# Kaz-K/medical-image-editing

Hardware: AMD Instinct MI355X
Metric: images/sec (train step, 256x256 2D slices) (higher is better)
Workload: dtype f32

## Files before the change

### medical-image-editing_amd/csrc/conv_common.h

```cpp
#pragma once
#include "common.h"
#include <cstdlib>

inline int conv_max_blocks() {
    static const int v = [] {
        const char* e = getenv("VQW_CONV_MAX_BLOCKS");
        const int b = e ? atoi(e) : 256;
        return b < 8 ? 8 : (b > 256 ? 256 : b);
    }();
    return v;
}

inline int conv_slab_split(int nsp, int nblk, int max_slabs, int* kt_out) {
    int nsb = conv_max_blocks() / nblk;
    if (nsb > max_slabs) nsb = max_slabs;
    if (nsb > nsp) nsb = nsp;
    if (nsb < 1) nsb = 1;
    const int kt = (nsp + nsb - 1) / nsb;
    if (kt_out) *kt_out = kt;
    return (nsp + kt - 1) / kt;
}
inline int conv_region_runs(int nsp, int ntn, int wg_per_cu) {
    int groups = conv_max_blocks() * wg_per_cu / ntn;
    if (groups < 1) groups = 1;
    const int even = (nsp + groups - 1) / groups;
    return even < 1 ? 1 : even;
}

struct ConvIn {
    const float* src0;
    const float* src1;
    int C0, C1, up0;
};

#ifdef __HIPCC__
static __device__ inline void collapse_up_element(const float* __restrict__ w, float* __restrict__ wc, float* __restrict__ wd, long i, int Cout, int Cin) {
    const long nfwd = 4L * Cout * 4 * Cin;
    if (i < nfwd) {
            int ci = (int)(i % Cin);
            long r = i / Cin;
            int ab = (int)(r % 4);
            r /= 4;
            int co = (int)(r % Cout);
            int par = (int)(r / Cout);
            int py = par >> 1, px = par & 1, a = ab >> 1, b = ab & 1;
            int ky0 = (py == 0) ? (a == 0 ? 0 : 1) : (a == 0 ? 0 : 2), ky1 = (py == 0) ? (a == 0 ? 0 : 2) : (a == 0 ? 1 : 2);
            int kx0 = (px == 0) ? (b == 0 ? 0 : 1) : (b == 0 ? 0 : 2), kx1 = (px == 0) ? (b == 0 ? 0 : 2) : (b == 0 ? 1 : 2);
            float acc = 0.f;
            for (int ky = ky0; ky <= ky1; ++ky)
                for (int kx = kx0; kx <= kx1; ++kx) acc += w[(((long)co * 3 + ky) * 3 + kx) * Cin + ci];
            wc[i] = acc;
        } else {
            long k = i - nfwd;
            int co = (int)(k % Cout);
            long r = k / Cout;
            int rs = (int)(r % 16);
            int ci = (int)(r / 16);
            int rr = rs >> 2, ss = rs & 3;
            int ky0 = rr == 0 ? 2 : (rr == 1 ? 1 : 0), ky1 = rr == 0 ? 2 : (rr == 1 ? 2 : (rr == 2 ? 1 : 0));
            int kx0 = ss == 0 ? 2 : (ss == 1 ? 1 : 0), kx1 = ss == 0 ? 2 : (ss == 1 ? 2 : (ss == 2 ? 1 : 0));
            float acc = 0.f;
            for (int ky = ky0; ky <= ky1; ++ky)
                for (int kx = kx0; kx <= kx1; ++kx) acc += w[(((long)co * 3 + ky) * 3 + kx) * Cin + ci];
            wd[k] = acc;
        }
}
// ... 142 lines not shown
```

### medical-image-editing_amd/csrc/conv_dil.hip

```cpp
#include "common.h"
#include "conv_common.h"
#include "mfma_util.h"

int g_dil_mode = 0;

namespace {

struct DilArgs {
    const float* x;
    const float* w;
    const float* bias;
    float* y;
    int N, H, W, Cout, dil;
    int per, total;
    int relu;
    unsigned nbx, nbw, nby;
    float* stats;
};

template <int NW, bool ACC>
__global__ void __launch_bounds__(64 * NW, 1) k_conv_dilrow(DilArgs a) {
    constexpr int NT = 64 * NW, WMAX = 32 * NW, KP = 36;
    constexpr int SLOT = (WMAX + 1) * KP;
    constexpr int WBUF = 9 * 32 * KP;
    constexpr int LH = WMAX * 8 / NT;
    constexpr int WF = 9 * 32 * 8, LW = (WF + NT - 1) / NT;
    static_assert(LH * NT == WMAX * 8, "row float4s must divide over the threads");

    extern __shared__ __attribute__((aligned(16))) float smem[];
    float* Hs = smem;
    float* Ws = smem + 3 * SLOT;
    float* Rs = Ws + WBUF;

    const int tid = threadIdx.x, lane = tid & 63, wv = tid >> 6;
    const int H = a.H, W = a.W, Cout = a.Cout, d = a.dil;
    const __amdgpu_buffer_rsrc_t rsx = make_rsrc(a.x, a.nbx), rsw = make_rsrc(a.w, a.nbw), rsy = make_rsrc(a.y, a.nby);

    const int t0 = blockIdx.x * a.per;
    const int nsteps = min(a.per, a.total - t0);
    if (nsteps <= 0) return;

    if (tid < 3 * KP) Hs[(tid / KP) * SLOT + WMAX * KP + tid % KP] = 0.f;
#pragma unroll
    for (int j = 0; j < LW; ++j) {
        const int f = tid + j * NT;
        const bool ok = (WF % NT == 0) || f < WF;
        const int row = ok ? f / 8 : 0, c4 = f % 8;
        const int tap = row / 32, n = row % 32;
        const float4 v = buf_ld4(rsw, (ok && n < Cout) ? (((unsigned)n * 9 + tap) * 32 + c4 * 4) * 4u : a.nbw);
        if (ok) *(float4*)&Ws[row * KP + c4 * 4] = v;
    }

    const unsigned row_bytes = (unsigned)W * 128u;
    unsigned h_off[LH];
    int h_lds[LH];
#pragma unroll
    for (int j = 0; j < LH; ++j) {
        const int f = tid + j * NT;
        h_off[j] = f < W * 8 ? (unsigned)f * 16u : 0xFFFFFFFFu;
        h_lds[j] = (f >> 3) * KP + (f & 7) * 4;
    }
    float4 rh[LH];
    auto issue_h = [&](int j, int g) {
        const bool ok = (g >= 0) & (h_off[j] != 0xFFFFFFFFu);
        rh[j] = buf_ld4(rsx, sel_u32(ok, (unsigned)g * row_bytes + h_off[j], a.nbx));
    };
    auto commit_h = [&](int j, int slot_f) { *(float4*)&Hs[slot_f + h_lds[j]] = rh[j]; };
    int hn, hrho, hy;
    if (t0 == 0) {
        hn = -1; hrho = d - 1; hy = -1;
    } else {
        const int Ls = H + d;
        hn = (t0 - 1) / Ls;
        int u = (t0 - 1) - hn * Ls;
        hrho = 0;
        for (;;) {
            const int L = (H - hrho + d - 1) / d;
            if (u < L) { hy = hrho + u * d; break; }
            if (u == L) { hy = -1; break; }
            u -= L + 1;
            ++hrho;
        }
    }
    auto head_row = [&]() { return (hy >= 0 && hn >= 0 && hn < a.N) ? hn * H + hy : -1; };
    auto head_next = [&]() {
        if (hy < 0) {
            if (++hrho == d) { hrho = 0; ++hn; }
            hy = hrho;
        } else {
            hy += d;
            if (hy >= H) hy = -1;
        }
    };

    int g0 = -1, g1 = -1;
#pragma unroll
    for (int s = 0; s < 3; ++s) {
        const int g = head_row();
#pragma unroll
        for (int j = 0; j < LH; ++j) issue_h(j, g);
#pragma unroll
        for (int j = 0; j < LH; ++j) commit_h(j, s * SLOT);
        head_next();
        g0 = g1;
        g1 = g;
    }
    int sA = 0, sB = SLOT, sC = 2 * SLOT;
    __syncthreads();

    const int lrow = lane & 31, lk = (lane >> 5) * 4;
    auto col_of = [&](int kx) {
        const int x = wv * 32 + lrow + (kx - 1) * d;
        return ((unsigned)x < (unsigned)W ? x : WMAX) * KP + lk;
    };
    const int cx0 = col_of(0), cx1 = col_of(1), cx2 = col_of(2);
    const float* Wb = Ws + lrow * KP + lk;

    const int co = lane & 31;
    const float bv0 = (a.bias && co < Cout) ? a.bias[co] : 0.f;
    const bool st_ok = (co < Cout) & (wv * 32 < W);
    const int col0 = 4 * (lane >> 5);
    const float lo = a.relu ? 0.f : -__builtin_inff();
    f32x16 acc, done;
    float yold[ACC ? 16 : 1];
    bool pending = false;
    int dg = 0;
    auto flush_piece = [&](int half) {
        const unsigned base = (((unsigned)dg * W + (unsigned)(wv * 32 + col0)) * (unsigned)Cout + (unsigned)co) * 4u;
        const int voff = (int)sel_u32(pending & st_ok, base, a.nby);
#pragma unroll
        for (int r8 = 0; r8 < 8; ++r8) {
            const int r = half * 8 + r8;
            const int col = (r & 3) + 8 * (r >> 2);
            __builtin_amdgcn_raw_buffer_store_b32(__float_as_uint(done[r]), rsy, voff, col * Cout * 4, 0);
        }
    };
    const int nwr = W / 32;

    for (int i = 0; i < nsteps; ++i) {
        const int g2 = (i + 2 <= nsteps) ? head_row() : -1;
        if (g0 >= 0) {
#pragma unroll
            for (int r = 0; r < 16; ++r) acc[r] = 0.f;
            constexpr int NG = 36;
            float4 av[2], bv[2];
            auto ldfrag = [&](int g, int s) {
                const int tap = g / 4, kg = g % 4, ky = tap / 3, kx = tap % 3;
                av[s] = *(const float4*)&Hs[(ky == 0 ? sA : ky == 1 ? sB : sC) + (kx == 0 ? cx0 : kx == 1 ? cx1 : cx2) + kg * 8];
                bv[s] = *(const float4*)&Wb[tap * 32 * KP + kg * 8];
            };
            auto slot = [&](int m) {
                if (m < 2) flush_piece(m);
                else if (m < 2 + LH) issue_h(m - 2, g2);
                else if (ACC && m < 2 + LH + 16) {
                    const int r = m - 2 - LH;
                    const unsigned base = (((unsigned)g0 * W + (unsigned)(wv * 32 + col0)) * (unsigned)Cout + (unsigned)co) * 4u;
                    yold[r] = __uint_as_float(__builtin_amdgcn_raw_buffer_load_b32(rsy, (int)sel_u32(st_ok, base, a.nby),
                                                                                 ((r & 3) + 8 * (r >> 2)) * Cout * 4, 0));
                }
                else if (m >= 96 && m < 96 + LH) commit_h(m - 96, sA);
            };
            auto slotted = [&](int m0) { return m0 >= 0 && (m0 < 2 + LH + (ACC ? 16 : 0) || (m0 + 4 > 96 && m0 < 96 + LH)); };
            ldfrag(0, 0);
#pragma unroll
            for (int g = 0; g < NG; ++g) {
                const int s = g & 1;
                if (g + 1 < NG) ldfrag(g + 1, s ^ 1);
                const int m0 = (g - 1) * 4;
                const bool slt = slotted(m0);
                acc = MFMA32(av[s].x, bv[s].x, acc);
                if (slt) { slot(m0); __builtin_amdgcn_sched_barrier(0); }
                acc = MFMA32(av[s].y, bv[s].y, acc);
                if (slt) { slot(m0 + 1); __builtin_amdgcn_sched_barrier(0); }
                acc = MFMA32(av[s].z, bv[s].z, acc);
                if (slt) { slot(m0 + 2); __builtin_amdgcn_sched_barrier(0); }
                acc = MFMA32(av[s].w, bv[s].w, acc);
                if (slt) { slot(m0 + 3); __builtin_amdgcn_sched_barrier(0); }
                if (!slt) {
                    __builtin_amdgcn_sched_group_barrier(0x100, 2, 0);
                    __builtin_amdgcn_sched_group_barrier(0x008, 4, 0);
                }
                if (g == 11) __syncthreads();
            }
            pending = false;
#pragma unroll
            for (int r = 0; r < 16; ++r) done[r] = fmaxf(acc[r] + bv0, lo) + (ACC ? yold[r] : 0.f);
            pending = true;
            dg = g0;
            if (a.stats) {
                float vals[16], s1, s2;
#pragma unroll
                for (int r = 0; r < 16; ++r) vals[r] = done[r];
                lane_stats<16>(vals, s1, s2);
                stat_merge_eq(s1, s2, __shfl_xor(s1, 32, 64), __shfl_xor(s2, 32, 64), 1.f / 32.f);
                if (lane < 32) { Rs[(wv * 32 + lane) * 2] = s1; Rs[(wv * 32 + lane) * 2 + 1] = s2; }
            }
        } else {
#pragma unroll
            for (int j = 0; j < LH; ++j) issue_h(j, g2);
#pragma unroll
            for (int j = 0; j < LH; ++j) commit_h(j, sA);
        }
        __syncthreads();
        if (a.stats && g0 >= 0 && tid < 32 && tid < Cout) {
            float s1 = Rs[tid * 2], s2 = Rs[tid * 2 + 1];
            for (int r = 1; r < nwr; ++r) stat_merge(s1, s2, (float)(32 * r), Rs[(r * 32 + tid) * 2], Rs[(r * 32 + tid) * 2 + 1], 32.f);
            float* o = a.stats + ((size_t)g0 * Cout + tid) * 2;
            o[0] = s1;
            o[1] = s2;
        }
        const int t = sA; sA = sB; sB = sC; sC = t;
        g0 = g1; g1 = g2;
        head_next();
    }
    flush_piece(0);
    flush_piece(1);
}


struct DilWgArgs {
    const float* x;
    const float* dy;
    float* part;
    int N, H, W, Cout, dil;
    int per, total;
    unsigned nbx, nbd;
};

template <int NW>
__global__ void __launch_bounds__(64 * NW, 1) k_conv_dilrow_wgrad(DilWgArgs a) {
    constexpr int NT = 64 * NW, WMAX = 32 * NW;
    constexpr int LH = WMAX * 8 / NT;
    extern __shared__ __attribute__((aligned(16))) float smem[];
    float* Xs = smem;

// ... 230 lines not shown
```

### medical-image-editing_amd/csrc/conv_wino64.hip

```cpp
#include "common.h"
#include "conv_common.h"
#include "mfma_util.h"
#include "wino_common.h"

extern int g_wino_mode;

namespace {

struct W64Args {
    const float* x;
    const float* u;
    const float* bias;
    float* y;
    int N, H, W, Cin, Cout;
    int tilesY, tilesX, nsp;
    int ntn, nch;
    int kt;
    int relu;
    unsigned nbx, nbu, nby;
    float* stats;
    const float* mask;
    const float* mr;
    int in_relu;
    float* y2;
// ... 43 lines not shown
    float* Rs = Ex + G::EXF;

    const int tid = threadIdx.x, lane = tid & 63;
    const int wv = __builtin_amdgcn_readfirstlane(tid >> 6);
    const int mb = wv & (NMB - 1), h = wv / NMB;
    const int H = a.H, W = a.W, Cin = a.Cin, Cout = a.Cout;
    const __amdgpu_buffer_rsrc_t rsx = make_rsrc(a.x, a.nbx), rsu = make_rsrc(a.u, a.nbu), rsy = make_rsrc(a.y, a.nby);
    const __amdgpu_buffer_rsrc_t rsm = make_rsrc((EPI == 1 || EPI == 3) ? a.mask : a.y, a.nby);
    const __amdgpu_buffer_rsrc_t rsr = make_rsrc(EPI == 3 ? a.mr : a.y, EPI == 3 ? (unsigned)((size_t)a.N * a.Cout * 8) : a.nby);
    const __amdgpu_buffer_rsrc_t rsy2 = make_rsrc(EPI == 4 ? a.y2 : a.y, EPI == 4 ? a.nby2 : a.nby);

    const int nch = a.nch;
    const wino::RegionRun run = wino::region_run(a.ntn, a.kt, a.nsp);
    const int co_base = run.tile_n * NCO;
    const int my_tiles = run.my_tiles;
    if (my_tiles <= 0) return;

    const int c4 = tid & 1;
    const wino::PitchedPix pixel = {a.img_px, a.rowb_px, a.rpx, a.ppx, a.n_sh, a.n_m};
    Halo hs;
    hs.init(tid, pixel);
    auto region_offsets = [&](int n, int tx, int ty) { hs.region_offsets(n, ty * G::TR - 1, tx * RW - 1, H, W, Cin); };
    const int u_n = (tid >> 1) & (NCO - 1);
    const int u_swz = (u_n >> 3) & 1;
    const int u_c4 = c4 ^ u_swz;
    const unsigned u_voff = (((unsigned)(tid >> 1) / NCO * Cout + co_base + u_n) * 8u + u_c4 * 4) * 4u;
    const unsigned u_jstride = (unsigned)(NT / 2 / NCO) * Cout * 32u;
    const unsigned u_cstride = 16u * Cout * 32u;
    const int u_wave = wv * 256;

    auto issue_h = [&](int j, int chunk) { hs.issue_h(rsx, j, chunk); };
    auto commit_h = [&](int j, float* Hb) { hs.commit_h(j, Hb); };
    auto issue_u = [&](int j, int chunk, float* Ub) {
        wino::buf_ld4_lds(rsu, Ub + u_wave + j * (NT * 4), u_voff, chunk * u_cstride + j * u_jstride);
    };

    int cn, ctx, cty, ch = 0;
    region_start(run.sp0, a.tilesY, a.tilesX, cn, ctx, cty);
    auto advance = [&](int& n, int& tx, int& ty, int& c) {
        const int adv = c + 1 == nch ? 1 : 0;
        c = adv ? 0 : c + 1;
        region_step(adv, a.tilesY, a.tilesX, n, tx, ty);
    };
    int n1 = cn, tx1 = ctx, ty1 = cty, ch1 = 0;
    advance(n1, tx1, ty1, ch1);
    int n2 = n1, tx2 = tx1, ty2 = ty1, ch2 = ch1;
    advance(n2, tx2, ty2, ch2);
    auto shift = [&]() {
        cn = n1; ctx = tx1; cty = ty1; ch = ch1;
        n1 = n2; tx1 = tx2; ty1 = ty2; ch1 = ch2;
        advance(n2, tx2, ty2, ch2);
    };

    const int m = lane & 15, q = lane >> 4;
    const int rA = h ? 3 : 0, rB = h ? 2 : 1, rC = h ? 1 : 2;
    const int prow = RW == 32 ? 2 * MBW * mb : 2 * (2 * mb + (m >> 3)), pcol = RW == 32 ? 2 * m : 2 * (m & 7);
    constexpr int MBW_STEP = 2 * HWS * W6_KPH;
    const int a_A = opaque(((prow + rA) * HWS + pcol) * W6_KPH + 2 * q);
    const int a_B = opaque(((prow + rB) * HWS + pcol) * W6_KPH + 2 * q);
    const int a_C = opaque(((prow + rC) * HWS + pcol) * W6_KPH + 2 * q);
    const int b_swz = ((q >> 1) ^ (m >> 3)) * 4 + (q & 1) * 2;
    const int b_0 = opaque(((h ? 3 : 0) * 4 * NCO + m) * 8 + b_swz);
    const int b_1 = opaque(((h ? 2 : 1) * 4 * NCO + m) * 8 + b_swz);
    const float sg = opaque_f(h ? -1.f : 1.f), mone = opaque_f(-1.f);

    f32x4 acc[8][MBW][NBW];
    f32x2 bf[2][NBW];
// ... 15 lines not shown
            else e[t][1][c] = __builtin_fmaf(sg, dC, dB);
        } else {
            const int k = o - 16, lr = k >> 3, t = (k >> 2) & 1, cc = k & 3;
            const float e0 = e[t][lr][0], e1 = e[t][lr][1], e2 = e[t][lr][2], e3 = e[t][lr][3];
            v[par][w][t][lr * 4 + cc] = wino::bt_row_plain(cc, e0, e1, e2, e3);
        }
    };
    auto xform_slot = [&](const float* Hn, int par, int p) {
        constexpr int NOPS = 32 * MBW, P0 = MBW == 1 ? 32 : 4;
        auto op = [&](int g) { xform_op(par, g >> 5, g & 31); };
        auto rd = [&](int g) {
            if ((g & 31) < 16 && ((g & 31) & 3) == 0) read_col(Hn, g >> 5, (g & 31) >> 2);
        };
        if (p + 3 - P0 >= 0 && p + 3 - P0 < NOPS) rd(p + 3 - P0);
        if (p - P0 >= 0 && p - P0 < NOPS && p < 64) {
            const int g = p - P0;
            if (P0 + NOPS <= 64 || g < NOPS - 2 * (P0 + NOPS - 64)) op(g);
            else { const int d = g - (NOPS - 2 * (P0 + NOPS - 64)); op(NOPS - 2 * (P0 + NOPS - 64) + 2 * d); op(NOPS - 2 * (P0 + NOPS - 64) + 2 * d + 1); }
        }
    };

    region_offsets(cn, ctx, cty);
#pragma unroll
    for (int j = 0; j < LH; ++j) issue_h(j, 0);
#pragma unroll
    for (int j = 0; j < LU; ++j) issue_u(j, 0, Us);
#pragma unroll
    for (int j = 0; j < LH; ++j) commit_h(j, Hs);
    region_offsets(n1, tx1, ty1);
#pragma unroll
    for (int j = 0; j < LH; ++j) issue_h(j, ch1);
#pragma unroll
    for (int j = 0; j < LH; ++j) commit_h(j, Hs + HBUF);
    wino::dma_wait();
    __syncthreads();
#pragma unroll
    for (int w = 0; w < MBW; ++w)
#pragma unroll
        for (int o = 0; o < 32; ++o) {
            if (o < 16 && (o & 3) == 0) read_col(Hs, w, o >> 2);
            xform_op(0, w, o);
        }
    __syncthreads();
    region_offsets(n2, tx2, ty2);

    float bvv[NBW / 2];
#pragma unroll
    for (int i = 0; i < NBW / 2; ++i) bvv[i] = a.bias ? a.bias[co_base + (h * (NBW / 2) + i) * 16 + m] : 0.f;
    const float lo = a.relu ? 0.f : -__builtin_inff();
    const bool plain = a.bias == nullptr && !a.relu;
    int spar = 0;

    auto body = [&](auto PAR, auto FIRST) {
        constexpr int par = decltype(PAR)::value;
        constexpr bool first = decltype(FIRST)::value;
        const float* Uc = Us + par * UBUF;
        const float* Hn = Hs + (par ^ 1) * HBUF;
        float* Hw = Hs + par * HBUF;
        float* Uw = Us + (par ^ 1) * UBUF;
        auto ldb = [&](int l, int nb) {
            bf[l & 1][nb] = *(const f32x2*)&Uc[(l < 4 ? b_0 : b_1) + ((l & 3) * NCO + nb * 16) * 8];
        };
        static_assert(par == 0 || (par ^ 1) == 0, "a region's last item (odd) loads U into buffer 0: buffer 1 is the epilogue's exchange area");
        auto slot = [&](int p) {
            if (p >= 1 && p < HP0 && (p - 1) % W6_ULS == 0) issue_u((p - 1) / W6_ULS, ch1, Uw);
            if (p >= HP0 && p < HP0 + LH * W6_LS && (p - HP0) % W6_LS == 0) issue_h((p - HP0) / W6_LS, ch2);
            if (p >= W6_CP && p < W6_CP + LH) commit_h(p - W6_CP, Hw);
// ... 175 lines not shown
        if (a.stats && lane < 16) {
#pragma unroll
            for (int i = 0; i < NBW / 2; ++i) {
                float* R = Rs + spar * (NMB * NCO * 2) + (mb * NCO + (hh * (NBW / 2) + i) * 16 + lane) * 2;
                R[0] = st1[i];
                R[1] = st2[i];
            }
        }
    };
    auto fold_stats = [&]() {
        if (!a.stats) return;
        if (tid < NCO) {
            const float* R = Rs + spar * (NMB * NCO * 2) + tid * 2;
            float s1 = R[0], s2 = R[1];
            constexpr float PW = 64.f * MBW;
            if (EPI == 3) {
#pragma unroll
                for (int r = 1; r < NMB; ++r) { s1 += R[r * NCO * 2]; s2 += R[r * NCO * 2 + 1]; }
            } else {
#pragma unroll
                for (int r = 1; r < NMB; ++r) stat_merge(s1, s2, PW * r, R[r * NCO * 2], R[r * NCO * 2 + 1], PW);
            }
            const int t = (cn * a.tilesX + ctx) * a.tilesY + cty;
            float* o = a.stats + ((size_t)t * Cout + co_base + tid) * 2;
            o[0] = s1;
            o[1] = s2;
        }
        spar ^= 1;
    };

    using wino::P0;
    using wino::P1;
    auto item_end = [&]() {
        wino::dma_wait();
        __syncthreads();
    };
    for (int reg = 0; reg < my_tiles; ++reg) {
        body(P0{}, std::true_type{});
        item_end();
        shift();
        body(P1{}, std::false_type{});
        item_end();
        for (int c = 2; c < nch; c += 2) {
            shift();
            if (ch2 == 0) region_offsets(n2, tx2, ty2);
            body(P0{}, std::false_type{});
            item_end();
            shift();
            body(P1{}, std::false_type{});
            item_end();
        }
        flush();
        if (h == 0) epi_send(P0{}); else epi_send(P1{});
        __syncthreads();
        if (h == 0) epi_finish(P0{}); else epi_finish(P1{});
        __syncthreads();
        fold_stats();
        shift();
        if (ch2 == 0) region_offsets(n2, tx2, ty2);
    }
}

}

static int wino64_shape(int Cin, int Cout, int W) {
    if (Cin % 16 != 0) return 0;
    if (Cout % 64 == 0) return 1;
// ... 450 lines not shown
```

### medical-image-editing_amd/csrc/conv_wino_up.hip

```cpp
#include "common.h"
#include "conv_common.h"
#include "mfma_util.h"
#include "wino_common.h"

namespace {

__device__ __host__ constexpr int up_row(int s) { return s == 2 ? 3 : s; }

__global__ void k_wino_up_weights(const float* __restrict__ w, float* __restrict__ uf, float* __restrict__ ud, int Cout, int Cin,
                                  float* __restrict__ wc, float* __restrict__ wd) {
    if (wc) {
        const long nc = 32L * Cout * Cin;
        for (long i = (long)blockIdx.x * blockDim.x + threadIdx.x; i < nc; i += (long)gridDim.x * blockDim.x) collapse_up_element(w, wc, wd, i, Cout, Cin);
    }
    const long n = (long)Cout * Cin;
    for (long e = (long)blockIdx.x * blockDim.x + threadIdx.x; e < n; e += (long)gridDim.x * blockDim.x) {
        const int co = (int)(e / Cin), ci = (int)(e % Cin);
        double g[3][3];
        for (int ky = 0; ky < 3; ++ky)
            for (int kx = 0; kx < 3; ++kx) g[ky][kx] = (double)w[(((long)co * 3 + ky) * 3 + kx) * Cin + ci];
        for (int flip = 0; flip < 2; ++flip) {
            double gf[3][3], u[4][4];
            for (int ky = 0; ky < 3; ++ky)
                for (int kx = 0; kx < 3; ++kx) gf[ky][kx] = flip ? g[2 - ky][2 - kx] : g[ky][kx];
// ... 8 lines not shown
                        const double ci_ = (i == 0 ? 1.0 : i == 1 ? 2.0 : -1.0), cj_ = (j == 0 ? 1.0 : j == 1 ? 2.0 : -1.0);
                        ud[((((long)(co >> 3) * 9 + xi) * Cin + ci) * 8) + (co & 7)] = (float)(ci_ * cj_ * u[i][j]);
                    }
                }
        }
    }
}

constexpr int WU_KPH = 10;

struct WUpDgArgs {
    const float* dy;
    const float* u;
    float* g;
    int N, H, W, Cin, Cout;
    int tilesY, tilesX, nsp, ntn, nch, kt;
    unsigned nbd, nbu, nbg;
};

template <int NBW, bool ACC>
__global__ void __launch_bounds__(512, 1) k_conv_wino_up_dgrad(WUpDgArgs a) {
    constexpr int NT = 512, NCO = 16 * NBW;
    constexpr int RW = 32, TR = 16, HR = TR + 2, HWV = RW + 2, HWS = 34;
    constexpr int HBUF = HR * HWS * WU_KPH;
    constexpr int UBUF = 9 * NCO * 8;
    using Halo = wino::HaloStager<NT, HR, HWV, HWS, wino::DensePix>;
    constexpr int LH = Halo::LH;
    constexpr int UF = 9 * NCO * 2;
    constexpr int LU = (UF + NT - 1) / NT;
    constexpr int NPOS = 18 * NBW;
    constexpr int NOPS = 42;
    constexpr int OPSTEP2 = NBW == 8 ? 3 : 2;
    constexpr int T0 = NPOS - (NOPS * OPSTEP2 + 1) / 2;
    constexpr int CP = T0 - (LH + LU) - 4;
    static_assert(1 + 2 * (LH + LU) <= CP, "prefetch loads are issued before their commits");

    extern __shared__ __attribute__((aligned(16))) float smem[];

    const int tid = threadIdx.x, lane = tid & 63;
    const int wv = __builtin_amdgcn_readfirstlane(tid >> 6);
    const int H = a.H, W = a.W, Cin = a.Cin, Cout = a.Cout;
    const __amdgpu_buffer_rsrc_t rsd = make_rsrc(a.dy, a.nbd), rsu = make_rsrc(a.u, a.nbu), rsg = make_rsrc(a.g, a.nbg);

    const int nch = a.nch;
    const wino::RegionRun run = wino::region_run(a.ntn, a.kt, a.nsp);
    const int co_base = run.tile_n * NCO;
    const int my_tiles = run.my_tiles;
    if (my_tiles <= 0) return;

    const int c4 = tid & 1;
    Halo hs;
    hs.init(tid, wino::DensePix{(unsigned)H, (unsigned)W});
    auto region_offsets = [&](int n, int tx, int ty) { hs.region_offsets(n, ty * TR - 1, tx * RW - 1, H, W, Cout); };
    unsigned u_voff[LU];
    int u_lds[LU];
#pragma unroll
    for (int j = 0; j < LU; ++j) {
        int f = tid + j * NT;
        if (f >= UF) f -= UF;
        const int row = f >> 1, xi = row / NCO, n = row - xi * NCO;
        u_voff[j] = (((unsigned)xi * Cin + co_base + n) * 8u + c4 * 4) * 4u;
        u_lds[j] = 2 * HBUF + row * 8 + ((c4 ^ ((n >> 3) & 1)) * 4);
    }
    const unsigned u_cstride = 9u * Cin * 32u;

    float4 ru[LU];
    auto issue_h = [&](int j, int chunk) { hs.issue_h(rsd, j, chunk); };
    auto issue_u = [&](int j, int chunk) { ru[j] = buf_ld4(rsu, u_voff[j], __builtin_amdgcn_readfirstlane(chunk * u_cstride)); };
    auto commit_h = [&](int j, int buf) { hs.commit_h(j, smem + buf * HBUF); };
    auto commit_u = [&](int j, int buf) { *(float4*)&smem[u_lds[j] + buf * UBUF] = ru[j]; };

    wino::ItemCursor it(a, run.sp0);

    const int m = lane & 15, q = lane >> 4;
    int a_row[4];
#pragma unroll
    for (int r = 0; r < 4; ++r) a_row[r] = opaque(((2 * wv + r) * HWS + 2 * m) * WU_KPH + 2 * q);
    const int b_swz = ((q >> 1) ^ (m >> 3)) * 4 + (q & 1) * 2;
    const int b_u0 = opaque((2 * HBUF + m * 8 + b_swz) / 2), b_u1 = opaque((2 * HBUF + UBUF + m * 8 + b_swz) / 2);
    const float mone = opaque_f(-1.f), pone = opaque_f(1.f);

    f32x4 acc[NBW];
    f32x2 bf[2][NBW];
    f32x2 dcol[2][4];
    float e[2][3][4];
    float v[2][2][9];

    auto read_col = [&](int buf, int c) {
        const float* Hc = smem + buf * HBUF + c * WU_KPH;
#pragma unroll
        for (int r = 0; r < 4; ++r) dcol[c & 1][r] = *(const f32x2*)&Hc[a_row[r]];
    };
    auto xform_op = [&](int par, int o) {
        if (o < 24) {
            const int c = o / 6, t = (o % 6) / 3, s = o % 3;
            const float d0 = dcol[c & 1][0][t], d1 = dcol[c & 1][1][t], d2 = dcol[c & 1][2][t], d3 = dcol[c & 1][3][t];
            e[t][s][c] = wino::bt_row(up_row(s), d0, d1, d2, d3, pone, mone);
        } else {
            const int k = o - 24, t = k / 9, s = (k % 9) / 3, sj = k % 3;
            const float e0 = e[t][s][0], e1 = e[t][s][1], e2 = e[t][s][2], e3 = e[t][s][3];
            v[par][t][s * 3 + sj] = wino::bt_row(up_row(sj), e0, e1, e2, e3, pone, mone);
        }
    };
    auto op_pos = [](int o) { return T0 + (o * OPSTEP2) / 2; };
    auto xform_slot = [&](int buf, int par, int p) {
#pragma unroll
        for (int o = 0; o < NOPS; ++o) {
            if (o < 24 && o % 6 == 0 && op_pos(o) - 3 == p) read_col(buf, o / 6);
            if (op_pos(o) == p) xform_op(par, o);
        }
    };

    region_offsets(it.cn, it.ctx, it.cty);
#pragma unroll
    for (int j = 0; j < LH; ++j) issue_h(j, 0);
#pragma unroll
    for (int j = 0; j < LU; ++j) issue_u(j, 0);
#pragma unroll
    for (int j = 0; j < LH; ++j) commit_h(j, 0);
#pragma unroll
    for (int j = 0; j < LU; ++j) commit_u(j, 0);
    region_offsets(it.n1, it.tx1, it.ty1);
#pragma unroll
    for (int j = 0; j < LH; ++j) issue_h(j, it.ch1);
#pragma unroll
    for (int j = 0; j < LH; ++j) commit_h(j, 1);
    __syncthreads();
#pragma unroll
    for (int o = 0; o < NOPS; ++o) {
        if (o < 24 && o % 6 == 0) read_col(0, o / 6);
        xform_op(0, o);
    }
    __syncthreads();
    region_offsets(it.n2, it.tx2, it.ty2);

    auto body = [&](auto PAR, auto FIRST) {
        constexpr int par = decltype(PAR)::value;
        constexpr bool first = decltype(FIRST)::value;
        auto ldb = [&](int xi, int nb) {
            bf[xi & 1][nb] = ((const f32x2*)smem)[(par ? b_u1 : b_u0) + (xi * NCO + nb * 16) * 4];
        };
        auto slot = [&](int p) {
            if (p >= 1 && p < 1 + 2 * LH && (p & 1)) issue_h((p - 1) >> 1, it.ch2);
            if (p >= 1 + 2 * LH && p < 1 + 2 * (LH + LU) && (p & 1)) issue_u((p - 1 - 2 * LH) >> 1, it.ch1);
            if (p >= CP && p < CP + LH) commit_h(p - CP, par);
            if (p >= CP + LH && p < CP + LH + LU) commit_u(p - CP - LH, par ^ 1);
            xform_slot(par ^ 1, par ^ 1, p);
        };
#pragma unroll
        for (int nb = 0; nb < NBW; ++nb) { ldb(0, nb); __builtin_amdgcn_sched_barrier(0); }
        const f32x4 zero4 = {0.f, 0.f, 0.f, 0.f};
#pragma unroll
        for (int xi = 0; xi < 9; ++xi)
#pragma unroll
            for (int k = 0; k < 2; ++k)
#pragma unroll
                for (int nb = 0; nb < NBW; ++nb) {
                    if (k == 0 && xi + 1 < 9) ldb(xi + 1, nb);
                    acc[nb] = MFMA16(v[par][k][xi], k == 0 ? bf[xi & 1][nb].x : bf[xi & 1][nb].y,
                                     (first && xi == 0 && k == 0) ? zero4 : acc[nb]);
                    slot((xi * 2 + k) * NBW + nb);
                    __builtin_amdgcn_sched_barrier(0);
                }
    };
    auto epilogue = [&]() {
        const int ylow = it.cty * (TR / 2) + wv, xlow0 = it.ctx * (RW / 2) + 4 * q;
        const unsigned base = (((unsigned)it.cn * (H >> 1) + (unsigned)ylow) * (W >> 1) + (unsigned)xlow0) * (unsigned)Cin + co_base + m;
        const int voff = (int)sel_u32(ylow < (H >> 1), base * 4u, 0xFFFFFFFFu);
        if (ACC) {
            float old[NBW][4];
#pragma unroll
            for (int nb = 0; nb < NBW; ++nb)
#pragma unroll
                for (int r = 0; r < 4; ++r) old[nb][r] = __uint_as_float(__builtin_amdgcn_raw_buffer_load_b32(rsg, voff, r * Cin * 4 + nb * 64, 0));
#pragma unroll
            for (int nb = 0; nb < NBW; ++nb)
#pragma unroll
                for (int r = 0; r < 4; ++r) acc[nb][r] = old[nb][r] + acc[nb][r];
        }
#pragma unroll
        for (int nb = 0; nb < NBW; ++nb)
#pragma unroll
            for (int r = 0; r < 4; ++r)
                __builtin_amdgcn_raw_buffer_store_b32(__float_as_uint(acc[nb][r]), rsg, voff, r * Cin * 4 + nb * 64, 0);
    };

    wino::region_loop(my_tiles, nch, it, body, region_offsets, epilogue);
}


struct WUpFwArgs {
    const float* x;
    const float* u;
    const float* bias;
    float* y;
    int N, h, w, Cin, Cout;
    int tilesY, tilesX, nsp, ntn, nch, kt;
    int relu;
    unsigned nbx, nbu, nby;
    float* stats;
    float* y2;
    float* stats2;
};

constexpr int WF_KPH = 12;

__global__ void __launch_bounds__(512, 1) k_conv_wino_up_fwd(WUpFwArgs a) {
    constexpr int NT = 512, NBW = 4, NCO = 64;
    constexpr int LR = 10, LWV = 18, LWS = 18;
    constexpr int HBUF = LR * LWS * WF_KPH;
    constexpr int UBUF = 9 * NCO * 8;
    constexpr int HF = LR * LWV * 2;
    constexpr int UF = 9 * NCO * 2;
    constexpr int LU = (UF + NT - 1) / NT;
    constexpr int NPOS = 72, NOPS = 24, T0 = NPOS - NOPS, CP = 30;
    static_assert(HF <= NT && 1 + 2 * (1 + LU) <= CP && CP + 1 + LU <= T0 - 3, "slot layout");

    extern __shared__ __attribute__((aligned(16))) float smem[];
    float* Rs = smem + 2 * HBUF + 2 * UBUF;

    const int tid = threadIdx.x, lane = tid & 63;
    const int wv = __builtin_amdgcn_readfirstlane(tid >> 6);
    const int h = a.h, w = a.w, Cin = a.Cin, Cout = a.Cout;
    const __amdgpu_buffer_rsrc_t rsx = make_rsrc(a.x, a.nbx), rsu = make_rsrc(a.u, a.nbu), rsy = make_rsrc(a.y, a.nby);
    const bool split = a.y2 != nullptr;
    const __amdgpu_buffer_rsrc_t rsy2 = make_rsrc(split ? a.y2 : a.y, a.nby);
    const int Cst = split ? 32 : a.Cout;

    const int nch = a.nch;
    const wino::RegionRun run = wino::region_run(a.ntn, a.kt, a.nsp);
    const int co_base = run.tile_n * NCO;
    const int my_tiles = run.my_tiles;
    if (my_tiles <= 0) return;

    const int c4 = tid & 1;
    const int hf = tid < HF ? tid : tid - HF;
    const int h_hy = (hf >> 1) / LWV, h_hx = (hf >> 1) - h_hy * LWV;
    const int h_lds = (h_hy * LWS + h_hx) * WF_KPH + c4 * 4;
    unsigned h_voff;
    auto region_offsets = [&](int n, int tx, int ty) {
        const int yy = ty * 8 - 1 + h_hy, xx = tx * 16 - 1 + h_hx;
        const bool ok = ((unsigned)yy < (unsigned)h) & ((unsigned)xx < (unsigned)w);
        const unsigned pix = ((unsigned)n * h + (unsigned)yy) * w + (unsigned)xx;
        h_voff = sel_u32(ok, pix * (unsigned)Cin * 4u + (unsigned)c4 * 16u, 0xFFFFFFFFu);
    };
    unsigned u_voff[LU];
    int u_lds[LU];
#pragma unroll
    for (int j = 0; j < LU; ++j) {
        int f = tid + j * NT;
        if (f >= UF) f -= UF;
        const int row = f >> 1, xi = row / NCO, n = row - xi * NCO;
        u_voff[j] = (((unsigned)xi * Cout + co_base + n) * 8u + c4 * 4) * 4u;
        u_lds[j] = 2 * HBUF + row * 8 + ((c4 ^ ((n >> 3) & 1)) * 4);
    }
    const unsigned u_cstride = 9u * Cout * 32u;

    float4 rh, ru[LU];
    auto issue_h = [&](int chunk) { rh = buf_ld4(rsx, h_voff, chunk * 32); };
    auto issue_u = [&](int j, int chunk) { ru[j] = buf_ld4(rsu, u_voff[j], __builtin_amdgcn_readfirstlane(chunk * u_cstride)); };
    auto commit_h = [&](int buf) { *(float4*)&smem[buf * HBUF + h_lds] = rh; };
    auto commit_u = [&](int j, int buf) { *(float4*)&smem[u_lds[j] + buf * UBUF] = ru[j]; };

    wino::ItemCursor it(a, run.sp0);

    const int m = lane & 15, q = lane >> 4;
    int a_row[3];
#pragma unroll
    for (int r = 0; r < 3; ++r) a_row[r] = opaque((((wv + r) * LWS + m) * WF_KPH + 2 * q) / 2);
    const int b_swz = ((q >> 1) ^ (m >> 3)) * 4 + (q & 1) * 2;
    const int b_u0 = opaque((2 * HBUF + m * 8 + b_swz) / 2), b_u1 = opaque((2 * HBUF + UBUF + m * 8 + b_swz) / 2);
    const float mone = opaque_f(-1.f);

    f32x4 acc[9][NBW];
    f32x2 bf[2][NBW];
    f32x2 dcol[2][3];
    float rr[2][3][3];
    float v[2][2][9];

    auto read_col = [&](int buf, int c) {
        const f32x2* Hc = (const f32x2*)smem + (buf * HBUF + c * WF_KPH) / 2;
#pragma unroll
        for (int r = 0; r < 3; ++r) dcol[c & 1][r] = Hc[a_row[r]];
    };
    auto xform_op = [&](int par, int o) {
        if (o < 12) {
            const int c = o / 4, t = (o % 4) / 2;
            const float da = dcol[c & 1][0][t], db = dcol[c & 1][1][t], dc = dcol[c & 1][2][t];
            if ((o & 1) == 0) { rr[t][0][c] = __builtin_fmaf(mone, db, da); rr[t][1][c] = db; }
            else rr[t][2][c] = __builtin_fmaf(mone, dc, db);
        } else {
            const int k = o - 12, t = k / 6, s = (k % 6) / 2;
            const float l = rr[t][s][0], mm = rr[t][s][1], r = rr[t][s][2];
            if ((o & 1) == 0) { v[par][t][s * 3 + 0] = __builtin_fmaf(mone, mm, l); v[par][t][s * 3 + 1] = mm; }
            else v[par][t][s * 3 + 2] = __builtin_fmaf(mone, r, mm);
        }
    };
    auto xform_slot = [&](int buf, int par, int p) {
#pragma unroll
        for (int o = 0; o < NOPS; ++o) {
            if (o < 12 && o % 4 == 0 && T0 + o - 3 == p) read_col(buf, o / 4);
            if (T0 + o == p) xform_op(par, o);
        }
    };

    region_offsets(it.cn, it.ctx, it.cty);
    issue_h(0);
#pragma unroll
    for (int j = 0; j < LU; ++j) issue_u(j, 0);
    commit_h(0);
#pragma unroll
    for (int j = 0; j < LU; ++j) commit_u(j, 0);
    region_offsets(it.n1, it.tx1, it.ty1);
    issue_h(it.ch1);
    commit_h(1);
    __syncthreads();
#pragma unroll
    for (int o = 0; o < NOPS; ++o) {
        if (o < 12 && o % 4 == 0) read_col(0, o / 4);
        xform_op(0, o);
    }
    __syncthreads();
    region_offsets(it.n2, it.tx2, it.ty2);

    float bvv[NBW];
#pragma unroll
    for (int nb = 0; nb < NBW; ++nb) bvv[nb] = a.bias ? a.bias[co_base + nb * 16 + m] : 0.f;
    const float lo = a.relu ? 0.f : -__builtin_inff();
    int spar = 0;

    auto body = [&](auto PAR, auto FIRST) {
        constexpr int par = decltype(PAR)::value;
        constexpr bool first = decltype(FIRST)::value;
        auto ldb = [&](int xi, int nb) {
            bf[xi & 1][nb] = ((const f32x2*)smem)[(par ? b_u1 : b_u0) + (xi * NCO + nb * 16) * 4];
        };
        auto slot = [&](int p) {
            if (p == 1) issue_h(it.ch2);
            if (p >= 3 && p < 3 + 2 * LU && (p & 1)) issue_u((p - 3) >> 1, it.ch1);
            if (p == CP) commit_h(par);
            if (p > CP && p <= CP + LU) commit_u(p - CP - 1, par ^ 1);
            xform_slot(par ^ 1, par ^ 1, p);
        };
#pragma unroll
        for (int nb = 0; nb < NBW; ++nb) { ldb(0, nb); __builtin_amdgcn_sched_barrier(0); }
        const f32x4 zero4 = {0.f, 0.f, 0.f, 0.f};
#pragma unroll
        for (int xi = 0; xi < 9; ++xi)
#pragma unroll
            for (int k = 0; k < 2; ++k)
#pragma unroll
                for (int nb = 0; nb < NBW; ++nb) {
                    if (k == 0 && xi + 1 < 9) ldb(xi + 1, nb);
                    acc[xi][nb] = MFMA16(v[par][k][xi], k == 0 ? bf[xi & 1][nb].x : bf[xi & 1][nb].y, (first && k == 0) ? zero4 : acc[xi][nb]);
                    slot((xi * 2 + k) * NBW + nb);
                    __builtin_amdgcn_sched_barrier(0);
                }
    };
    auto epilogue = [&]() {
        const int yrow0 = it.cty * 16 + 2 * wv, xcol0 = it.ctx * 32 + 8 * q;
        const int H = 2 * h, W = 2 * w;
#pragma unroll
        for (int nb = 0; nb < NBW; ++nb) {
            float yv[16];
#pragma unroll
            for (int r = 0; r < 4; ++r) {
                float t0[3], t1[3];
#pragma unroll
                for (int j = 0; j < 3; ++j) {
                    t0[j] = acc[j][nb][r] + acc[3 + j][nb][r];
                    t1[j] = acc[3 + j][nb][r] - acc[6 + j][nb][r];
                }
                yv[r * 4 + 0] = fmaxf((t0[0] + t0[1]) + bvv[nb], lo);
                yv[r * 4 + 1] = fmaxf((t0[1] - t0[2]) + bvv[nb], lo);
                yv[r * 4 + 2] = fmaxf((t1[0] + t1[1]) + bvv[nb], lo);
                yv[r * 4 + 3] = fmaxf((t1[1] - t1[2]) + bvv[nb], lo);
            }
            const bool second = split && nb >= 2;
            const unsigned co = second ? (unsigned)((nb - 2) * 16 + m) : (unsigned)(co_base + nb * 16 + m);
            const __amdgpu_buffer_rsrc_t rso = second ? rsy2 : rsy;
#pragma unroll
            for (int aa = 0; aa < 2; ++aa) {
                const int yy = yrow0 + aa;
                const unsigned base = (((unsigned)it.cn * H + (unsigned)yy) * W + (unsigned)xcol0) * (unsigned)Cst + co;
                const int voff = (int)sel_u32(yy < H, base * 4u, 0xFFFFFFFFu);
#pragma unroll
                for (int r = 0; r < 4; ++r)
#pragma unroll
                    for (int b = 0; b < 2; ++b)
                        __builtin_amdgcn_raw_buffer_store_b32(__float_as_uint(yv[r * 4 + aa * 2 + b]), rso, voff, (2 * r + b) * Cst * 4, 0);
// ... 403 lines not shown
```

### medical-image-editing_amd/csrc/wino_common.h

```cpp
#pragma once
#include "mfma_util.h"
#include <type_traits>

namespace wino {

using P0 = std::integral_constant<int, 0>;
using P1 = std::integral_constant<int, 1>;

struct RegionRun {
    int tile_n, sp0, my_tiles;
};
__device__ __forceinline__ RegionRun region_run(int ntn, int kt, int nsp) {
    const int lb = xcd_remap(blockIdx.x, gridDim.x);
    RegionRun r;
    r.tile_n = lb % ntn;
    r.sp0 = (lb / ntn) * kt;
    r.my_tiles = min(kt, nsp - r.sp0);
    return r;
}

template <class Args>
struct ItemCursor {
    const Args& a;
    int cn, ctx, cty, ch;
// ... 73 lines not shown
        const int hp = f >> 1;
        hy = hp / HWV;
        hx = hp - hy * HWV;
    }
    __device__ __forceinline__ void init(int tid_, const Pix& pix_) {
        tid = tid_; c4 = tid_ & 1; pix = pix_;
#pragma unroll
        for (int j = 0; j < LH; ++j) {
            int hy, hx;
            halo_pixel(j, hy, hx);
            h_lds[j] = (hy * HWS + hx) * KPH + c4 * 4;
        }
    }
    __device__ __forceinline__ void region_offsets(int n, int y0, int x0, int H, int W, int C) {
#pragma unroll
        for (int j = 0; j < LH; ++j) {
            int hy, hx;
            halo_pixel(j, hy, hx);
            const int yy = y0 + hy, xx = x0 + hx;
            const bool ok = ((unsigned)yy < (unsigned)H) & ((unsigned)xx < (unsigned)W);
            h_voff[j] = sel_u32(ok, pix(n, yy, xx) * (unsigned)C * 4u + (unsigned)c4 * 16u, 0xFFFFFFFFu);
        }
    }
    __device__ __forceinline__ void issue_h(__amdgpu_buffer_rsrc_t rs, int j, int chunk) { rh[j] = buf_ld4(rs, h_voff[j], chunk * 32); }
    __device__ __forceinline__ void commit_h(int j, float* Hb) {
        float* p = Hb + h_lds[j];
        f32x2 lo, hi;
        lo.x = rh[j].x; lo.y = rh[j].y; hi.x = rh[j].z; hi.y = rh[j].w;
        *(f32x2*)p = lo;
        *(f32x2*)(p + 2) = hi;
    }
};

__device__ __forceinline__ void buf_ld4_lds(__amdgpu_buffer_rsrc_t r, float* lds_wave, unsigned byte_off, unsigned soff) {
    __builtin_amdgcn_raw_ptr_buffer_load_lds(r, (__attribute__((address_space(3))) void*)lds_wave, 16, (int)byte_off, (int)soff, 0, 0);
}
__device__ __forceinline__ void dma_wait() { __builtin_amdgcn_s_waitcnt(0x0F70); }

__device__ __forceinline__ float bt_row(int r, float d0, float d1, float d2, float d3, float pone, float mone) {
    return r == 0 ? __builtin_fmaf(mone, d2, d0) : r == 1 ? __builtin_fmaf(pone, d2, d1) : r == 2 ? __builtin_fmaf(mone, d1, d2) : __builtin_fmaf(mone, d3, d1);
}
__device__ __forceinline__ float bt_row_plain(int r, float d0, float d1, float d2, float d3) {
    return r == 0 ? d0 - d2 : r == 1 ? d1 + d2 : r == 2 ? d2 - d1 : d1 - d3;
}

__device__ __forceinline__ void weight_transform(const double g[3][3], double u[4][4]) {
    double t[4][3];
    for (int kx = 0; kx < 3; ++kx) {
        t[0][kx] = g[0][kx];
        t[1][kx] = 0.5 * (g[0][kx] + g[1][kx] + g[2][kx]);
        t[2][kx] = 0.5 * (g[0][kx] - g[1][kx] + g[2][kx]);
        t[3][kx] = g[2][kx];
    }
    for (int i = 0; i < 4; ++i) {
        u[i][0] = t[i][0];
        u[i][1] = 0.5 * (t[i][0] + t[i][1] + t[i][2]);
        u[i][2] = 0.5 * (t[i][0] - t[i][1] + t[i][2]);
        u[i][3] = t[i][2];
    }
}

}
```

Measured before the change: 362.7.

## Stage dilated-conv rows and Winograd-up weights via direct buffer-to-LDS loads

Replaces register-staged global loads followed by LDS stores with buffer_load ... lds DMA in the dilated row conv (halo rows) and in both Winograd upsample kernels (U weight tiles). The LDS layout of the dilated halo is changed so each wave writes a contiguous run, and the XOR swizzle is moved to the global offset side. This removes VGPR staging and commit slots from the software pipeline and reorders the prefetch slots, at the cost of a dma_wait before each barrier and loading some padding lanes. The shared helpers move to conv_common.h.

```diff
diff --git a/medical-image-editing_amd/csrc/conv_common.h b/medical-image-editing_amd/csrc/conv_common.h
--- a/medical-image-editing_amd/csrc/conv_common.h
+++ b/medical-image-editing_amd/csrc/conv_common.h
@@ -32,6 +32,13 @@
     const float* src1;
     int C0, C1, up0;
 };
+
+#ifdef __HIPCC__
+__device__ __forceinline__ void buf_ld4_lds(__amdgpu_buffer_rsrc_t r, float* lds_wave, unsigned byte_off, unsigned soff) {
+    __builtin_amdgcn_raw_ptr_buffer_load_lds(r, (__attribute__((address_space(3))) void*)lds_wave, 16, (int)byte_off, (int)soff, 0, 0);
+}
+__device__ __forceinline__ void dma_wait() { __builtin_amdgcn_s_waitcnt(0x0F70); }
+#endif
 
 #ifdef __HIPCC__
 static __device__ inline void collapse_up_element(const float* __restrict__ w, float* __restrict__ wc, float* __restrict__ wd, long i, int Cout, int Cin) {
diff --git a/medical-image-editing_amd/csrc/conv_dil.hip b/medical-image-editing_amd/csrc/conv_dil.hip
--- a/medical-image-editing_amd/csrc/conv_dil.hip
+++ b/medical-image-editing_amd/csrc/conv_dil.hip
@@ -23,9 +23,11 @@
     constexpr int NT = 64 * NW, WMAX = 32 * NW, KP = 36;
     constexpr int SLOT = (WMAX + 1) * KP;
     constexpr int WBUF = 9 * 32 * KP;
-    constexpr int LH = WMAX * 8 / NT;
+    constexpr int Q = KP / 4;
+    constexpr int RF = WMAX * Q;
+    constexpr int LH = (RF + NT - 1) / NT;
     constexpr int WF = 9 * 32 * 8, LW = (WF + NT - 1) / NT;
-    static_assert(LH * NT == WMAX * 8, "row float4s must divide over the threads");
+    static_assert(RF >= NT, "a row takes at least one full slot");
 
     extern __shared__ __attribute__((aligned(16))) float smem[];
     float* Hs = smem;
@@ -33,6 +35,7 @@
     float* Rs = Ws + WBUF;
 
     const int tid = threadIdx.x, lane = tid & 63, wv = tid >> 6;
+    const int wvu = __builtin_amdgcn_readfirstlane(tid >> 6);
     const int H = a.H, W = a.W, Cout = a.Cout, d = a.dil;
     const __amdgpu_buffer_rsrc_t rsx = make_rsrc(a.x, a.nbx), rsw = make_rsrc(a.w, a.nbw), rsy = make_rsrc(a.y, a.nby);
 
@@ -51,21 +54,19 @@
         if (ok) *(float4*)&Ws[row * KP + c4 * 4] = v;
     }
 
+    auto row_f0 = [](int j) { return (j + 1) * NT <= RF ? j * NT : RF - NT; };
     const unsigned row_bytes = (unsigned)W * 128u;
     unsigned h_off[LH];
-    int h_lds[LH];
 #pragma unroll
     for (int j = 0; j < LH; ++j) {
-        const int f = tid + j * NT;
-        h_off[j] = f < W * 8 ? (unsigned)f * 16u : 0xFFFFFFFFu;
-        h_lds[j] = (f >> 3) * KP + (f & 7) * 4;
-    }
-    float4 rh[LH];
-    auto issue_h = [&](int j, int g) {
+        const int f = row_f0(j) + tid;
+        const int px = f / Q, q = f % Q;
+        h_off[j] = (q < 8 && px < W) ? (unsigned)px * 128u + (unsigned)q * 16u : 0xFFFFFFFFu;
+    }
+    auto issue_h = [&](int j, int g, int slot_f) {
         const bool ok = (g >= 0) & (h_off[j] != 0xFFFFFFFFu);
-        rh[j] = buf_ld4(rsx, sel_u32(ok, (unsigned)g * row_bytes + h_off[j], a.nbx));
-    };
-    auto commit_h = [&](int j, int slot_f) { *(float4*)&Hs[slot_f + h_lds[j]] = rh[j]; };
+        buf_ld4_lds(rsx, Hs + slot_f + (row_f0(j) + wvu * 64) * 4, sel_u32(ok, (unsigned)g * row_bytes + h_off[j], a.nbx), 0);
+    };
     int hn, hrho, hy;
     if (t0 == 0) {
         hn = -1; hrho = d - 1; hy = -1;
@@ -98,14 +99,13 @@
     for (int s = 0; s < 3; ++s) {
         const int g = head_row();
 #pragma unroll
-        for (int j = 0; j < LH; ++j) issue_h(j, g);
-#pragma unroll
-        for (int j = 0; j < LH; ++j) commit_h(j, s * SLOT);
+        for (int j = 0; j < LH; ++j) issue_h(j, g, s * SLOT);
         head_next();
         g0 = g1;
         g1 = g;
     }
     int sA = 0, sB = SLOT, sC = 2 * SLOT;
+    dma_wait();
     __syncthreads();
 
     const int lrow = lane & 31, lk = (lane >> 5) * 4;
@@ -143,24 +143,24 @@
 #pragma unroll
             for (int r = 0; r < 16; ++r) acc[r] = 0.f;
             constexpr int NG = 36;
-            float4 av[2], bv[2];
+            f32x4 av[2], bv[2];
             auto ldfrag = [&](int g, int s) {
                 const int tap = g / 4, kg = g % 4, ky = tap / 3, kx = tap % 3;
-                av[s] = *(const float4*)&Hs[(ky == 0 ? sA : ky == 1 ? sB : sC) + (kx == 0 ? cx0 : kx == 1 ? cx1 : cx2) + kg * 8];
-                bv[s] = *(const float4*)&Wb[tap * 32 * KP + kg * 8];
+                av[s] = *(const f32x4*)&Hs[(ky == 0 ? sA : ky == 1 ? sB : sC) + (kx == 0 ? cx0 : kx == 1 ? cx1 : cx2) + kg * 8];
+                bv[s] = *(const f32x4*)&Wb[tap * 32 * KP + kg * 8];
             };
+            constexpr int NOLD = ACC ? 16 : 0, LP = 44;
             auto slot = [&](int m) {
                 if (m < 2) flush_piece(m);
-                else if (m < 2 + LH) issue_h(m - 2, g2);
-                else if (ACC && m < 2 + LH + 16) {
-                    const int r = m - 2 - LH;
+                else if (ACC && m < 2 + NOLD) {
+                    const int r = m - 2;
                     const unsigned base = (((unsigned)g0 * W + (unsigned)(wv * 32 + col0)) * (unsigned)Cout + (unsigned)co) * 4u;
                     yold[r] = __uint_as_float(__builtin_amdgcn_raw_buffer_load_b32(rsy, (int)sel_u32(st_ok, base, a.nby),
                                                                                  ((r & 3) + 8 * (r >> 2)) * Cout * 4, 0));
                 }
-                else if (m >= 96 && m < 96 + LH) commit_h(m - 96, sA);
+                else if (m >= LP && m < LP + LH) issue_h(m - LP, g2, sA);
             };
-            auto slotted = [&](int m0) { return m0 >= 0 && (m0 < 2 + LH + (ACC ? 16 : 0) || (m0 + 4 > 96 && m0 < 96 + LH)); };
+            auto slotted = [&](int m0) { return m0 >= 0 && (m0 < 2 + NOLD || (m0 + 4 > LP && m0 < LP + LH)); };
             ldfrag(0, 0);
 #pragma unroll
             for (int g = 0; g < NG; ++g) {
@@ -197,10 +197,9 @@
             }
         } else {
 #pragma unroll
-            for (int j = 0; j < LH; ++j) issue_h(j, g2);
-#pragma unroll
-            for (int j = 0; j < LH; ++j) commit_h(j, sA);
-        }
+            for (int j = 0; j < LH; ++j) issue_h(j, g2, sA);
+        }
+        dma_wait();
         __syncthreads();
         if (a.stats && g0 >= 0 && tid < 32 && tid < Cout) {
             float s1 = Rs[tid * 2], s2 = Rs[tid * 2 + 1];
diff --git a/medical-image-editing_amd/csrc/conv_wino64.hip b/medical-image-editing_amd/csrc/conv_wino64.hip
--- a/medical-image-editing_amd/csrc/conv_wino64.hip
+++ b/medical-image-editing_amd/csrc/conv_wino64.hip
@@ -99,7 +99,7 @@
     auto issue_h = [&](int j, int chunk) { hs.issue_h(rsx, j, chunk); };
     auto commit_h = [&](int j, float* Hb) { hs.commit_h(j, Hb); };
     auto issue_u = [&](int j, int chunk, float* Ub) {
-        wino::buf_ld4_lds(rsu, Ub + u_wave + j * (NT * 4), u_voff, chunk * u_cstride + j * u_jstride);
+        buf_ld4_lds(rsu, Ub + u_wave + j * (NT * 4), u_voff, chunk * u_cstride + j * u_jstride);
     };
 
     int cn, ctx, cty, ch = 0;
@@ -181,7 +181,7 @@
     for (int j = 0; j < LH; ++j) issue_h(j, ch1);
 #pragma unroll
     for (int j = 0; j < LH; ++j) commit_h(j, Hs + HBUF);
-    wino::dma_wait();
+    dma_wait();
     __syncthreads();
 #pragma unroll
     for (int w = 0; w < MBW; ++w)
@@ -423,7 +423,7 @@
     using wino::P0;
     using wino::P1;
     auto item_end = [&]() {
-        wino::dma_wait();
+        dma_wait();
         __syncthreads();
     };
     for (int reg = 0; reg < my_tiles; ++reg) {
diff --git a/medical-image-editing_amd/csrc/conv_wino_up.hip b/medical-image-editing_amd/csrc/conv_wino_up.hip
--- a/medical-image-editing_amd/csrc/conv_wino_up.hip
+++ b/medical-image-editing_amd/csrc/conv_wino_up.hip
@@ -64,8 +64,8 @@
     constexpr int NOPS = 42;
     constexpr int OPSTEP2 = NBW == 8 ? 3 : 2;
     constexpr int T0 = NPOS - (NOPS * OPSTEP2 + 1) / 2;
-    constexpr int CP = T0 - (LH + LU) - 4;
-    static_assert(1 + 2 * (LH + LU) <= CP, "prefetch loads are issued before their commits");
+    constexpr int CP = T0 - LH - 4;
+    static_assert(1 + 2 * (LH + LU) <= CP, "prefetch loads are issued before the halo commits");
 
     extern __shared__ __attribute__((aligned(16))) float smem[];
 
@@ -84,23 +84,24 @@
     Halo hs;
     hs.init(tid, wino::DensePix{(unsigned)H, (unsigned)W});
     auto region_offsets = [&](int n, int tx, int ty) { hs.region_offsets(n, ty * TR - 1, tx * RW - 1, H, W, Cout); };
+    static_assert(UF % 64 == 0, "the wrap of the last U slot falls between waves");
     unsigned u_voff[LU];
-    int u_lds[LU];
 #pragma unroll
     for (int j = 0; j < LU; ++j) {
         int f = tid + j * NT;
         if (f >= UF) f -= UF;
         const int row = f >> 1, xi = row / NCO, n = row - xi * NCO;
-        u_voff[j] = (((unsigned)xi * Cin + co_base + n) * 8u + c4 * 4) * 4u;
-        u_lds[j] = 2 * HBUF + row * 8 + ((c4 ^ ((n >> 3) & 1)) * 4);
+        u_voff[j] = (((unsigned)xi * Cin + co_base + n) * 8u + (c4 ^ ((n >> 3) & 1)) * 4) * 4u;
     }
     const unsigned u_cstride = 9u * Cin * 32u;
 
-    float4 ru[LU];
     auto issue_h = [&](int j, int chunk) { hs.issue_h(rsd, j, chunk); };
-    auto issue_u = [&](int j, int chunk) { ru[j] = buf_ld4(rsu, u_voff[j], __builtin_amdgcn_readfirstlane(chunk * u_cstride)); };
+    auto issue_u = [&](int j, int chunk, int buf) {
+        const int f0 = wv * 64 + j * NT;
+        buf_ld4_lds(rsu, smem + 2 * HBUF + buf * UBUF + (f0 >= UF ? f0 - UF : f0) * 4, u_voff[j],
+                    __builtin_amdgcn_readfirstlane(chunk * u_cstride));
+    };
     auto commit_h = [&](int j, int buf) { hs.commit_h(j, smem + buf * HBUF); };
-    auto commit_u = [&](int j, int buf) { *(float4*)&smem[u_lds[j] + buf * UBUF] = ru[j]; };
 
     wino::ItemCursor it(a, run.sp0);
 
@@ -147,16 +148,15 @@
 #pragma unroll
     for (int j = 0; j < LH; ++j) issue_h(j, 0);
 #pragma unroll
-    for (int j = 0; j < LU; ++j) issue_u(j, 0);
+    for (int j = 0; j < LU; ++j) issue_u(j, 0, 0);
 #pragma unroll
     for (int j = 0; j < LH; ++j) commit_h(j, 0);
-#pragma unroll
-    for (int j = 0; j < LU; ++j) commit_u(j, 0);
     region_offsets(it.n1, it.tx1, it.ty1);
 #pragma unroll
     for (int j = 0; j < LH; ++j) issue_h(j, it.ch1);
 #pragma unroll
     for (int j = 0; j < LH; ++j) commit_h(j, 1);
+    dma_wait();
     __syncthreads();
 #pragma unroll
     for (int o = 0; o < NOPS; ++o) {
@@ -173,10 +173,9 @@
             bf[xi & 1][nb] = ((const f32x2*)smem)[(par ? b_u1 : b_u0) + (xi * NCO + nb * 16) * 4];
         };
         auto slot = [&](int p) {
-            if (p >= 1 && p < 1 + 2 * LH && (p & 1)) issue_h((p - 1) >> 1, it.ch2);
-            if (p >= 1 + 2 * LH && p < 1 + 2 * (LH + LU) && (p & 1)) issue_u((p - 1 - 2 * LH) >> 1, it.ch1);
+            if (p >= 1 && p < 1 + 2 * LU && (p & 1)) issue_u((p - 1) >> 1, it.ch1, par ^ 1);
+            if (p >= 1 + 2 * LU && p < 1 + 2 * (LU + LH) && (p & 1)) issue_h((p - 1 - 2 * LU) >> 1, it.ch2);
             if (p >= CP && p < CP + LH) commit_h(p - CP, par);
-            if (p >= CP + LH && p < CP + LH + LU) commit_u(p - CP - LH, par ^ 1);
             xform_slot(par ^ 1, par ^ 1, p);
         };
 #pragma unroll
@@ -194,6 +193,7 @@
                     slot((xi * 2 + k) * NBW + nb);
                     __builtin_amdgcn_sched_barrier(0);
                 }
+        dma_wait();
     };
     auto epilogue = [&]() {
         const int ylow = it.cty * (TR / 2) + wv, xlow0 = it.ctx * (RW / 2) + 4 * q;
@@ -246,7 +246,7 @@
     constexpr int UF = 9 * NCO * 2;
     constexpr int LU = (UF + NT - 1) / NT;
     constexpr int NPOS = 72, NOPS = 24, T0 = NPOS - NOPS, CP = 30;
-    static_assert(HF <= NT && 1 + 2 * (1 + LU) <= CP && CP + 1 + LU <= T0 - 3, "slot layout");
+    static_assert(HF <= NT && 1 + 2 * (1 + LU) <= CP && CP + 1 <= T0 - 3, "slot layout");
 
     extern __shared__ __attribute__((aligned(16))) float smem[];
     float* Rs = smem + 2 * HBUF + 2 * UBUF;
@@ -276,23 +276,28 @@
         const unsigned pix = ((unsigned)n * h + (unsigned)yy) * w + (unsigned)xx;
         h_voff = sel_u32(ok, pix * (unsigned)Cin * 4u + (unsigned)c4 * 16u, 0xFFFFFFFFu);
     };
+    static_assert(UF % 64 == 0, "the wrap of the last U slot falls between waves");
     unsigned u_voff[LU];
-    int u_lds[LU];
 #pragma unroll
     for (int j = 0; j < LU; ++j) {
         int f = tid + j * NT;
         if (f >= UF) f -= UF;
         const int row = f >> 1, xi = row / NCO, n = row - xi * NCO;
-        u_voff[j] = (((unsigned)xi * Cout + co_base + n) * 8u + c4 * 4) * 4u;
-        u_lds[j] = 2 * HBUF + row * 8 + ((c4 ^ ((n >> 3) & 1)) * 4);
+        u_voff[j] = (((unsigned)xi * Cout + co_base + n) * 8u + (c4 ^ ((n >> 3) & 1)) * 4) * 4u;
     }
     const unsigned u_cstride = 9u * Cout * 32u;
 
-    float4 rh, ru[LU];
+    float4 rh;
     auto issue_h = [&](int chunk) { rh = buf_ld4(rsx, h_voff, chunk * 32); };
-    auto issue_u = [&](int j, int chunk) { ru[j] = buf_ld4(rsu, u_voff[j], __builtin_amdgcn_readfirstlane(chunk * u_cstride)); };
-    auto commit_h = [&](int buf) { *(float4*)&smem[buf * HBUF + h_lds] = rh; };
-    auto commit_u = [&](int j, int buf) { *(float4*)&smem[u_lds[j] + buf * UBUF] = ru[j]; };
+    auto issue_u = [&](int j, int chunk, int buf) {
+        const int f0 = wv * 64 + j * NT;
+        buf_ld4_lds(rsu, smem + 2 * HBUF + buf * UBUF + (f0 >= UF ? f0 - UF : f0) * 4, u_voff[j],
+                    __builtin_amdgcn_readfirstlane(chunk * u_cstride));
+    };
+    auto commit_h = [&](int buf) {
+        const f32x4 t = {rh.x, rh.y, rh.z, rh.w};
+        *(f32x4*)&smem[buf * HBUF + h_lds] = t;
+    };
 
     wino::ItemCursor it(a, run.sp0);
 
@@ -339,13 +344,12 @@
     region_offsets(it.cn, it.ctx, it.cty);
     issue_h(0);
 #pragma unroll
-    for (int j = 0; j < LU; ++j) issue_u(j, 0);
+    for (int j = 0; j < LU; ++j) issue_u(j, 0, 0);
     commit_h(0);
-#pragma unroll
-    for (int j = 0; j < LU; ++j) commit_u(j, 0);
     region_offsets(it.n1, it.tx1, it.ty1);
     issue_h(it.ch1);
     commit_h(1);
+    dma_wait();
     __syncthreads();
 #pragma unroll
     for (int o = 0; o < NOPS; ++o) {
@@ -369,9 +373,8 @@
         };
         auto slot = [&](int p) {
             if (p == 1) issue_h(it.ch2);
-            if (p >= 3 && p < 3 + 2 * LU && (p & 1)) issue_u((p - 3) >> 1, it.ch1);
+            if (p >= 3 && p < 3 + 2 * LU && (p & 1)) issue_u((p - 3) >> 1, it.ch1, par ^ 1);
             if (p == CP) commit_h(par);
-            if (p > CP && p <= CP + LU) commit_u(p - CP - 1, par ^ 1);
             xform_slot(par ^ 1, par ^ 1, p);
         };
 #pragma unroll
@@ -388,6 +391,7 @@
                     slot((xi * 2 + k) * NBW + nb);
                     __builtin_amdgcn_sched_barrier(0);
                 }
+        dma_wait();
     };
     auto epilogue = [&]() {
         const int yrow0 = it.cty * 16 + 2 * wv, xcol0 = it.ctx * 32 + 8 * q;
diff --git a/medical-image-editing_amd/csrc/wino_common.h b/medical-image-editing_amd/csrc/wino_common.h
--- a/medical-image-editing_amd/csrc/wino_common.h
+++ b/medical-image-editing_amd/csrc/wino_common.h
@@ -129,11 +129,6 @@
     }
 };
 
-__device__ __forceinline__ void buf_ld4_lds(__amdgpu_buffer_rsrc_t r, float* lds_wave, unsigned byte_off, unsigned soff) {
-    __builtin_amdgcn_raw_ptr_buffer_load_lds(r, (__attribute__((address_space(3))) void*)lds_wave, 16, (int)byte_off, (int)soff, 0, 0);
-}
-__device__ __forceinline__ void dma_wait() { __builtin_amdgcn_s_waitcnt(0x0F70); }
-
 __device__ __forceinline__ float bt_row(int r, float d0, float d1, float d2, float d3, float pone, float mone) {
     return r == 0 ? __builtin_fmaf(mone, d2, d0) : r == 1 ? __builtin_fmaf(pone, d2, d1) : r == 2 ? __builtin_fmaf(mone, d1, d2) : __builtin_fmaf(mone, d3, d1);
 }
```

Result: no change. 362.6 (-0.0%).
